# q8888620002/Group-Attribution-for-Diffusion-Models

Measured on AMD Instinct MI355X. Metric: shapley_coalitions_per_hour, higher is better.
Workload: dtype f32; 1 GPU; CIFAR-20 DDPM sFT coalition (BASELINE configs[1]): gd_steps=1000 @B=128 + 10240 samples x 100 DDIM steps @B=32 (32 batches fused/launch), UNet2DModel widths [128, 256, 256, 256] 35.75M params fp32; step = 1/1000 coalition = 1 train step + 1 sampler step @B=1024, enqueued on 3 HIP streams (the train step belongs to a later coalition: independent work); coalitions_in_flight=3

## Files before the change

### group-attribution-for-diffusion-models_amd/csrc/gemm_f32.hip

```cpp
#include "gad_common.h"
#include "gemm_dev.h"

using namespace gadk;

namespace gadk {
void launch_wino4_fused(const DevArgs& w, int bm, hipStream_t st);
}

namespace {

template <int ROWS, int VEC>
struct LoadKCDense : KCSlots<ROWS> {
  using S = KCSlots<ROWS>;
  const float* base;
  long roff[S::NS];
  unsigned rowmask;
  int kend, k;
  bool kok;
  __device__ void init(const float* b, int ld, int row0, int nrows, int kend_) {
    base = b;
    kend = kend_;
    rowmask = 0;
#pragma unroll
    for (int i = 0; i < S::NS; ++i) {
// ... 2009 lines not shown
    amul(d, col);
#pragma unroll
    for (int i = 0; i < 6; ++i) t[i][dx] = col[i];
  }
  const long pos_stride = p.T * p.C;
  float* out = p.V + tile * p.C + c;
#pragma unroll
  for (int i = 0; i < 6; ++i) {
    f32x4 v[6];
    amul(t[i], v);
#pragma unroll
    for (int j = 0; j < 6; ++j) *reinterpret_cast<f32x4*>(out + (long)(6 * i + j) * pos_stride) = v[j];
  }
}

__global__ __launch_bounds__(256) void wino4_dw_kernel(const float* dU, float* dW, int Cout, int Cin, int ldc) {
  const int C4 = Cin >> 2;
  const long idx = (long)blockIdx.x * 256 + threadIdx.x;
  if (idx >= (long)Cout * C4) return;
  const int co = (int)(idx / C4), ci = (int)(idx - (long)co * C4) * 4;
  const long ps = (long)Cout * Cin;
  const float* src = dU + (long)co * Cin + ci;
  auto gt = [](const f32x4 (&m)[6], f32x4 (&o)[3]) {
    const f32x4 s12 = m[1] + m[2], d21 = m[2] - m[1], s34 = m[3] + m[4], d34 = m[3] - m[4];
    o[0] = 0.25f * m[0] - (1.f / 6.f) * s12 + (1.f / 24.f) * s34;
    o[1] = (1.f / 6.f) * d21 + (1.f / 12.f) * d34;
    o[2] = (1.f / 6.f) * (s34 - s12) + m[5];
  };
  f32x4 t[3][6];
#pragma unroll
  for (int nu = 0; nu < 6; ++nu) {
    f32x4 m[6], col[3];
#pragma unroll
    for (int xi = 0; xi < 6; ++xi) m[xi] = ldg4(src + (long)(6 * xi + nu) * ps);
    gt(m, col);
#pragma unroll
    for (int r = 0; r < 3; ++r) t[r][nu] = col[r];
  }
  float* dst = dW + (long)co * ldc + ci;
#pragma unroll
  for (int r = 0; r < 3; ++r) {
    f32x4 o[3];
    gt(t[r], o);
#pragma unroll
    for (int sx = 0; sx < 3; ++sx) *reinterpret_cast<f32x4*>(dst + (long)(r * 3 + sx) * Cin) = o[sx];
  }
}

static FastDiv make_fastdiv(unsigned d) {
// ... 314 lines not shown
  out->lda = g.ldx;
  if (a->A2) {
    out->A_k2 = a->A2; out->lda_k2 = a->ldx2;
    out->B_k2 = a->B + a->a_split; out->ldb_k2 = a->ldb;
    out->k_split = a->a_split;
    out->A2 = nullptr; out->a_split = 0;
  }
  return true;
}
static gad_gemm_args canonical(const gad_gemm_args* a) {
  gad_gemm_args c;
  return as_dense_1x1(a, &c) ? c : *a;
}

constexpr int GAD_GEMM_INTERNAL_WINO4 = 1 << 30;
struct WinoPlan {
  int f;
  int fused4;
  int bm, bn, tiles_m, tiles_n;
  long T;
  int64_t bytes;
};
static bool use_wino(const gad_gemm_args* a, WinoPlan* wp) {
  const gad_conv_geom& g = a->g;
  if ((!a->B_wino && !a->B_wino4) || a->operand_precision != 0 || a->a_mode != GAD_A_CONV || a->b_mode != GAD_B_KC || a->A2 || a->A_k2) return false;
  if (!same_3x3(g) || (g.Ho & 1) || (g.Wo & 1)) return false;
  if (g.C % BK != 0 || g.ldx % 4 != 0 || a->N % 4 != 0 || a->N < 64 || (a->tile_hint != 0 && (a->tile_hint < HINT_WINO2 || a->tile_hint > HINT_WINO4_FUSED64)) || a->splitk_hint > 0 || a->batch > 1) return false;
  if (a->flags & (GAD_GEMM_NO_WINO | GAD_GEMM_NO_PATCH | GAD_GEMM_SCALAR_EPILOGUE | GAD_GEMM_TAP_MAJOR_K)) return false;
  if (a->rowadd && a->rows_per_group != g.Ho * g.Wo) return false;
  if (a->M % (g.Ho * g.Wo) != 0) return false;
// ... 252 lines not shown
extern "C" int gad_wino_weights(const float* src, float* dst, const int64_t* table, int64_t n_tiles, void* stream) {
  GAD_CHECK(src && dst && table && n_tiles > 0 && n_tiles < (1L << 31), "gad_wino_weights: bad arguments");
  static_assert(sizeof(long) == sizeof(int64_t), "table rows are 64-bit");
  hipLaunchKernelGGL(wino_weights_kernel, dim3((unsigned)n_tiles), dim3(256), 0, (hipStream_t)stream, src, dst, (const long*)table);
  GAD_LAUNCH_CHECK("gad_wino_weights");
  return 0;
}

extern "C" int gad_wino4_weights(const float* src, float* dst, const int64_t* table, int64_t n_tiles, void* stream) {
  GAD_CHECK(src && dst && table && n_tiles > 0 && n_tiles < (1L << 31), "gad_wino4_weights: bad arguments");
  hipLaunchKernelGGL(wino4_weights_kernel, dim3((unsigned)n_tiles), dim3(256), 0, (hipStream_t)stream, src, dst, (const long*)table);
  GAD_LAUNCH_CHECK("gad_wino4_weights");
  return 0;
}


static int check_args(const gad_gemm_args* a) {
  GAD_CHECK(a->M > 0 && a->N > 0 && a->K > 0, "gad_gemm: bad shape M=%d N=%d K=%d", a->M, a->N, a->K);
  const int am = a->a_mode, bmode = a->b_mode;
  GAD_CHECK(gad_aligned16(a->A) && gad_aligned16(a->B), "gad_gemm: A/B must be 16-byte aligned");
  const int k_first = a->A_k2 ? a->k_split : a->K;
  if (am == GAD_A_KC) GAD_CHECK(a->lda >= k_first, "gad_gemm: A_KC needs lda >= K (K=%d lda=%d)", k_first, a->lda);
  if (am == GAD_A_MC) GAD_CHECK(a->lda >= a->M, "gad_gemm: A_MC needs lda >= M (M=%d lda=%d)", a->M, a->lda);
  if (bmode == GAD_B_KC) GAD_CHECK(a->ldb >= k_first, "gad_gemm: B_KC needs ldb >= K (K=%d ldb=%d)", k_first, a->ldb);
  if (bmode == GAD_B_MC) GAD_CHECK(a->ldb >= a->N, "gad_gemm: B_MC needs ldb >= N (N=%d ldb=%d)", a->N, a->ldb);
  const bool convA = am == GAD_A_CONV || am == GAD_A_CONVT;
  if (convA || bmode == GAD_B_CONV || bmode == GAD_B_WDGRAD) {
    const gad_conv_geom& g = a->g;
    GAD_CHECK(g.H > 0 && g.W > 0 && g.C > 0 && g.Ho > 0 && g.Wo > 0 && g.KH > 0 && g.KW > 0 && g.stride > 0 &&
              g.ldx >= (a->A2 ? a->a_split : g.C), "gad_gemm: bad conv geometry");
// ... 34 lines not shown
  }
  if (a->rowadd) GAD_CHECK(a->rows_per_group > 0 && a->ld_rowadd >= a->N, "gad_gemm: bad rowadd");
  if (a->residual) GAD_CHECK(a->ldr >= a->N, "gad_gemm: bad residual stride");
  GAD_CHECK(a->ldc >= a->N, "gad_gemm: ldc < N");
  GAD_CHECK(a->operand_precision == 0 || a->operand_precision == 1, "gad_gemm: operand_precision must be 0 (f32) or 1 (bf16 allowed)");
  return 0;
}

static int check_stage_flags(const Route& r) {
  const bool only_input = (r.a.flags & GAD_GEMM_WINO_ONLY_INPUT) != 0, skip_input = (r.a.flags & GAD_GEMM_WINO_SKIP_INPUT) != 0;
  GAD_CHECK(!(only_input && skip_input), "gad_gemm: GAD_GEMM_WINO_ONLY_INPUT and GAD_GEMM_WINO_SKIP_INPUT exclude each other");
  GAD_CHECK(!only_input || r.kind == RouteKind::WINO,
            "gad_gemm: GAD_GEMM_WINO_ONLY_INPUT on a launch that takes no Winograd forward route (kernel id %d)", report(r).kid);
  GAD_CHECK(!skip_input || r.kind == RouteKind::WINO || r.kind == RouteKind::WINO_WGRAD,
            "gad_gemm: GAD_GEMM_WINO_SKIP_INPUT on a launch that takes no Winograd route (kernel id %d)", report(r).kid);
  return 0;
}

static DevArgs dev_args(const gad_gemm_args* a) {
  DevArgs d;
  d.A = a->A; d.B = a->B; d.C = a->C;
  d.A2 = a->A2; d.a_split = a->a_split; d.ldx2 = a->ldx2;
  d.Ak2 = a->A_k2; d.Bk2 = a->B_k2; d.lda2 = a->lda_k2; d.ldb2 = a->ldb_k2; d.k_split = a->k_split;
  d.Bh = nullptr;
  d.M = a->M; d.N = a->N; d.K = a->K;
  d.lda = a->lda; d.ldb = a->ldb; d.ldc = a->ldc;
  d.batch_inner = a->batch_inner > 0 ? a->batch_inner : 1;
  d.sA0 = a->strideA0; d.sA1 = a->strideA1; d.sB0 = a->strideB0; d.sB1 = a->strideB1;
  d.sC0 = a->strideC0; d.sC1 = a->strideC1;
  d.g = a->g;
// ... 21 lines not shown
static int launch_wino_wgrad(const Route& r, void* stream) {
  const gad_gemm_args* a = &r.a;
  const WinoWgradPlan& wq = r.wq;
  const gad_conv_geom& g = a->g;
  hipStream_t st = (hipStream_t)stream;
  GAD_CHECK(a->wino_ws && a->wino_ws_bytes >= wq.bytes && gad_aligned16(a->wino_ws),
            "gad_gemm: Winograd weight-gradient workspace too small or misaligned (%lld < %lld)", (long long)a->wino_ws_bytes, (long long)wq.bytes);
  float* Wy = (float*)a->wino_ws;
  float* V = Wy + wq.wy_bytes / 4;
  float* dU = V + wq.v_bytes / 4;
  const bool have_v = (a->flags & GAD_GEMM_WINO_SKIP_INPUT) && a->B_wino4 != nullptr;
  if (have_v) {
    GAD_CHECK(gad_aligned16(a->B_wino4), "gad_gemm: the kept Winograd input image (B_wino4 of a weight-gradient launch) must be 16-byte aligned");
    V = const_cast<float*>(a->B_wino4);
  }
  WinoIn wy;
  wy.x = a->A; wy.V = Wy;
  wy.H = g.Ho; wy.W = g.Wo; wy.C = a->M; wy.ldx = a->lda; wy.up = 0;
  wy.TH = g.Ho / 4; wy.TW = g.Wo / 4; wy.T = wq.T;
  WinoIn wi;
  wi.x = a->B; wi.V = V;
  wi.H = g.H; wi.W = g.W; wi.C = g.C; wi.ldx = g.ldx; wi.up = g.upsample ? 1 : 0;
  wi.TH = wy.TH; wi.TW = wy.TW; wi.T = wq.T;
  const long iy = wq.T * (a->M / 4), ix = wq.T * (g.C / 4);
  GAD_CHECK(gad_ceil_div(iy, 256) < (1L << 31) && gad_ceil_div(ix, 256) < (1L << 31), "gad_gemm: Winograd transform grid too large");
  hipLaunchKernelGGL(wino4_dy_kernel, dim3((unsigned)gad_ceil_div(iy, 256)), dim3(256), 0, st, wy);
  if (!have_v) hipLaunchKernelGGL(wino4_input_kernel, dim3((unsigned)gad_ceil_div(ix, 256)), dim3(256), 0, st, wi);
  GAD_LAUNCH_CHECK("gad_gemm(winograd wgrad transforms)");
  const gad_gemm_args sub = wino_wgrad_products_args(a, wq, Wy, V, dU);
  if (const int rc = gad_gemm(&sub, stream)) return rc;
  const long items = (long)a->M * (g.C / 4);
  hipLaunchKernelGGL(wino4_dw_kernel, dim3((unsigned)gad_ceil_div(items, 256)), dim3(256), 0, st, dU, a->C, a->M, g.C, a->ldc);
  GAD_LAUNCH_CHECK("gad_gemm(winograd wgrad output transform)");
  return 0;
}

static int launch_wino(const Route& r, const DevArgs& d, void* stream) {
  const gad_gemm_args* a = &r.a;
  const WinoPlan& wp = r.wp;
  const gad_conv_geom& g = a->g;
  hipStream_t st = (hipStream_t)stream;
  GAD_CHECK(a->wino_ws && a->wino_ws_bytes >= wp.bytes && gad_aligned16(a->wino_ws) && gad_aligned16(wp.f == 2 ? a->B_wino : a->B_wino4),
            "gad_gemm: Winograd workspace too small or misaligned (%lld < %lld)", (long long)a->wino_ws_bytes, (long long)wp.bytes);
  WinoIn wi;
  wi.x = a->A; wi.V = (float*)a->wino_ws;
  wi.H = g.H; wi.W = g.W; wi.C = g.C; wi.ldx = g.ldx; wi.up = g.upsample ? 1 : 0;
  wi.TH = g.Ho / wp.f; wi.TW = g.Wo / wp.f; wi.T = wp.T;
// ... 218 lines not shown
    else if (vec == 4) launch_mode<AMODE, BMODE_, 4>(d, pl, st);                       \
    else launch_mode<AMODE, BMODE_, 1>(d, pl, st);                                     \
  } else
  GAD_CASE(GAD_A_KC, GAD_B_KC)
  GAD_CASE(GAD_A_KC, GAD_B_MC)
  GAD_CASE(GAD_A_MC, GAD_B_MC)
  GAD_CASE(GAD_A_CONV, GAD_B_KC)
  GAD_CASE(GAD_A_CONVT, GAD_B_WDGRAD)
  GAD_CASE(GAD_A_MC, GAD_B_CONV)
  {
    gad_set_error("gad_gemm: unsupported mode pair a_mode=%d b_mode=%d", am, bmode);
    return 1;
  }
#undef GAD_CASE
  GAD_LAUNCH_CHECK("gad_gemm");
  if (pl.splitk > 1) {
    launch_splitk_reduce(d, (int)batch, st);
    GAD_LAUNCH_CHECK("gad_gemm(splitk reduce)");
  }
  return 0;
}

extern "C" int gad_gemm(const gad_gemm_args* args, void* stream) {
  GAD_CHECK(args && args->A && args->B && args->C, "gad_gemm: null pointer");
  const gad_gemm_args canon = canonical(args);
  if (const int rc = check_args(&canon)) return rc;
  const Route r = route_of(&canon);
  if (const int rc = check_stage_flags(r)) return rc;
  hipStream_t st = (hipStream_t)stream;
  DevArgs d = dev_args(&r.a);
  switch (r.kind) {
// ... 17 lines not shown
```

### group-attribution-for-diffusion-models_amd/gad/_capi.py

```python
import ctypes as C
import os

_HERE = os.path.dirname(os.path.abspath(__file__))
LIB_PATH = os.path.join(_HERE, "libgad_hip.so")


class GadError(RuntimeError):
    pass


class ConvGeom(C.Structure):
    _fields_ = [("H", C.c_int32), ("W", C.c_int32), ("C", C.c_int32), ("ldx", C.c_int32),
                ("Ho", C.c_int32), ("Wo", C.c_int32), ("KH", C.c_int32), ("KW", C.c_int32),
                ("stride", C.c_int32), ("pad_t", C.c_int32), ("pad_l", C.c_int32), ("upsample", C.c_int32)]


class GemmArgs(C.Structure):
    _fields_ = [("A", C.c_void_p), ("B", C.c_void_p), ("C", C.c_void_p),
                ("a_mode", C.c_int32), ("b_mode", C.c_int32),
                ("M", C.c_int32), ("N", C.c_int32), ("K", C.c_int32),
                ("lda", C.c_int32), ("ldb", C.c_int32), ("ldc", C.c_int32),
                ("batch", C.c_int32), ("batch_inner", C.c_int32),
                ("strideA0", C.c_int64), ("strideA1", C.c_int64), ("strideB0", C.c_int64),
                ("strideB1", C.c_int64), ("strideC0", C.c_int64), ("strideC1", C.c_int64),
                ("g", ConvGeom),
                ("alpha", C.c_float), ("bias", C.c_void_p), ("rowadd", C.c_void_p),
                ("rows_per_group", C.c_int32), ("ld_rowadd", C.c_int32),
                ("residual", C.c_void_p), ("ldr", C.c_int32),
                ("ws", C.c_void_p), ("ws_bytes", C.c_int64),
                ("tile_hint", C.c_int32), ("splitk_hint", C.c_int32), ("operand_precision", C.c_int32),
                ("A2", C.c_void_p), ("a_split", C.c_int32), ("ldx2", C.c_int32), ("B_bf16", C.c_void_p),
                ("A_k2", C.c_void_p), ("B_k2", C.c_void_p), ("lda_k2", C.c_int32), ("ldb_k2", C.c_int32),
                ("k_split", C.c_int32), ("flags", C.c_int32),
                ("B_wino", C.c_void_p), ("wino_ws", C.c_void_p), ("wino_ws_bytes", C.c_int64), ("B_wino4", C.c_void_p)]


class GroupNormArgs(C.Structure):
    _fields_ = [("x", C.c_void_p), ("y", C.c_void_p), ("gamma", C.c_void_p), ("beta", C.c_void_p),
                ("mean", C.c_void_p), ("rstd", C.c_void_p), ("dy", C.c_void_p),
                ("dgamma", C.c_void_p), ("dbeta", C.c_void_p),
                ("B", C.c_int32), ("HW", C.c_int32), ("C", C.c_int32), ("G", C.c_int32),
                ("eps", C.c_float), ("silu", C.c_int32), ("ws", C.c_void_p), ("ws_bytes", C.c_int64),
                ("x2", C.c_void_p), ("C1", C.c_int32), ("flags", C.c_int32), ("dx_add", C.c_void_p)]


class AttentionArgs(C.Structure):
    _fields_ = [("q", C.c_void_p), ("k", C.c_void_p), ("v", C.c_void_p), ("o", C.c_void_p), ("lse", C.c_void_p),
                ("d_o", C.c_void_p), ("delta", C.c_void_p), ("dq", C.c_void_p), ("dk", C.c_void_p), ("dv", C.c_void_p),
                ("B", C.c_int32), ("heads", C.c_int32), ("Tq", C.c_int32), ("Tk", C.c_int32), ("d", C.c_int32),
# ... 38 lines not shown


class HGemmSegArgs(C.Structure):
    _fields_ = [("A", C.c_void_p), ("B", C.c_void_p), ("C", C.c_void_p), ("ws", C.c_void_p), ("ws_bytes", C.c_int64),
                ("c_seg_stride", C.c_int64), ("M", C.c_int32), ("N", C.c_int32), ("L", C.c_int32), ("S", C.c_int32),
                ("lda", C.c_int32), ("ldb", C.c_int32), ("ldc", C.c_int32), ("alpha", C.c_float), ("accumulate", C.c_int32),
                ("splitk_hint", C.c_int32)]


JL_NORMAL, JL_RADEMACHER = 0, 1

GEMM_NO_PATCH, GEMM_TAP_MAJOR_K, GEMM_SCALAR_EPILOGUE, GEMM_GENERAL_LOADERS, GN_TWO_PASS = 1, 2, 4, 8, 1
GEMM_NO_WINO = 16
GEMM_WINO_WGRAD = 32
GEMM_WINO_ONLY_INPUT, GEMM_WINO_SKIP_INPUT = 64, 128
A_KC, A_MC, A_CONV, A_CONVT = 0, 1, 2, 3
B_KC, B_MC, B_WDGRAD, B_CONV = 0, 1, 2, 3

_vp, _i32, _i64, _f32, _f64 = C.c_void_p, C.c_int32, C.c_int64, C.c_float, C.c_double

SIGNATURES = {
    "gad_version": (C.c_int, []),
    "gad_last_error": (C.c_char_p, []),
    "gad_gemm_workspace_bytes": (_i64, [C.POINTER(GemmArgs)]),
    "gad_gemm": (C.c_int, [C.POINTER(GemmArgs), _vp]),
    "gad_gemm_uses_bf16": (C.c_int, [C.POINTER(GemmArgs)]),
    "gad_gemm_kernel_id": (C.c_int, [C.POINTER(GemmArgs)]),
    "gad_gemm_wino_bytes": (_i64, [C.POINTER(GemmArgs)]),
    "gad_wino_weights": (C.c_int, [_vp, _vp, _vp, _i64, _vp]),
    "gad_wino4_weights": (C.c_int, [_vp, _vp, _vp, _i64, _vp]),
    "gad_groupnorm_one_pass": (C.c_int, [C.POINTER(GroupNormArgs)]),
    "gad_gemm_plan": (C.c_int, [C.POINTER(GemmArgs), C.POINTER(_i32), C.POINTER(_i32), C.POINTER(_i32)]),
    "gad_groupnorm_workspace_bytes": (_i64, [C.POINTER(GroupNormArgs)]),
    "gad_groupnorm_silu_fwd": (C.c_int, [C.POINTER(GroupNormArgs), _vp]),
    "gad_groupnorm_silu_bwd": (C.c_int, [C.POINTER(GroupNormArgs), _vp]),
    "gad_groupnorm_wino4_ok": (C.c_int, [C.POINTER(GroupNormArgs), C.c_int32]),
    "gad_groupnorm_silu_wino4": (C.c_int, [C.POINTER(GroupNormArgs), _vp, C.c_int32, _vp]),
    "gad_attention_supported": (C.c_int, [_i32]),
    "gad_attention_uses_bf16": (C.c_int, [C.POINTER(AttentionArgs), _i32]),
    "gad_attention_bwd_workspace_bytes": (_i64, [C.POINTER(AttentionArgs)]),
    "gad_attention_fwd": (C.c_int, [C.POINTER(AttentionArgs), _vp]),
    "gad_attention_bwd": (C.c_int, [C.POINTER(AttentionArgs), _vp]),
    "gad_softmax_fwd": (C.c_int, [_vp, _vp, _i64, _i32, _f32, _vp]),
    "gad_softmax_bwd": (C.c_int, [_vp, _vp, _vp, _i64, _i32, _f32, _vp]),
    "gad_layernorm_workspace_bytes": (_i64, [_i64, _i32]),
# ... 73 lines not shown
```

### group-attribution-for-diffusion-models_amd/gad/ops.py

```python
from __future__ import annotations

import ctypes as C
import math
from typing import Optional

import torch

from . import _capi
from ._capi import (A_CONV, A_CONVT, A_KC, A_MC, B_CONV, B_KC, B_MC, B_WDGRAD, AdamArgs, ConvGeom, GemmArgs,
                    GroupNormArgs, check)

_WS = {}
WS_BYTES = 1 << 30


def _stream():
    return C.c_void_p(torch.cuda.current_stream().cuda_stream)


_raw_stream = getattr(torch._C, "_cuda_getCurrentRawStream", None)


WS_OVERRIDE = [None]

# ... 85 lines not shown

    def __exit__(self, *exc):
        OPERAND_PRECISION[0] = self.prev
        return False


def set_operand_precision(name):
    OPERAND_PRECISION[0] = 0 if name in (None, "no", "f32", "fp32") else operand_precision("bf16" if name in ("fp16", "bf16") else name).value


def half_activations() -> bool:
    return OPERAND_PRECISION[0] == 2


KERNEL_FLAGS = {"gemm": 0, "gn": 0, "native_dgrad": False, "two_kernel_attn_bwd": False, "narrow_attn_fwd": False, "no_wino4": False,
                "no_gn_wino": False}


class kernel_flags:

    def __init__(self, no_patch=False, tap_major_k=False, gn_two_pass=False, scalar_epilogue=False, general_loaders=False,
                 native_dgrad=False, two_kernel_attn_bwd=False, narrow_attn_fwd=False, no_wino=False, no_wino4=False, no_gn_wino=False):
        self.native_dgrad, self.two_kernel_attn_bwd, self.narrow_attn_fwd, self.no_wino4 = native_dgrad, two_kernel_attn_bwd, narrow_attn_fwd, no_wino4
        self.no_gn_wino = no_gn_wino
        self.gemm = ((_capi.GEMM_NO_PATCH if no_patch else 0) | (_capi.GEMM_TAP_MAJOR_K if tap_major_k else 0)
                     | (_capi.GEMM_NO_WINO if no_wino else 0)
                     | (_capi.GEMM_SCALAR_EPILOGUE if scalar_epilogue else 0)
                     | (_capi.GEMM_GENERAL_LOADERS if general_loaders else 0))
        self.gn = _capi.GN_TWO_PASS if gn_two_pass else 0

    def __enter__(self):
        self.prev = dict(KERNEL_FLAGS)
        KERNEL_FLAGS["gemm"], KERNEL_FLAGS["gn"], KERNEL_FLAGS["native_dgrad"] = self.gemm, self.gn, self.native_dgrad
        KERNEL_FLAGS["two_kernel_attn_bwd"], KERNEL_FLAGS["narrow_attn_fwd"] = self.two_kernel_attn_bwd, self.narrow_attn_fwd
        KERNEL_FLAGS["no_wino4"] = self.no_wino4
        KERNEL_FLAGS["no_gn_wino"] = self.no_gn_wino
        return self

    def __exit__(self, *exc):
        KERNEL_FLAGS.update(self.prev)
        return False


SCRATCH_ALLOC = None
OUT_ALLOC = None
OUT_ALLOC_DT = None


ROUTE_STATS = None


# ... 1 lines not shown
    if SCRATCH_ALLOC is not None:
        return SCRATCH_ALLOC(kind, nbytes, device)
    return torch.empty(nbytes, dtype=torch.uint8, device=device)


def _out(shape, device):
    if OUT_ALLOC is not None:
        return OUT_ALLOC(tuple(shape), device)
    return torch.empty(tuple(shape), device=device, dtype=torch.float32)


def gemm_raw(A, B, Cout, a_mode, b_mode, M, N, K, lda, ldb, ldc, *, geom: Optional[ConvGeom] = None, alpha=1.0,
             bias=None, rowadd=None, rows_per_group=1, residual=None, ldr=0, batch=1, batch_inner=1,
             sA=(0, 0), sB=(0, 0), sC=(0, 0), tile_hint=0, splitk_hint=0, A2=None, a_split=0, B_bf16=None,
             A_k2=None, B_k2=None, k_split=0, B_wino=None, B_wino4=None, wino_wgrad=False, wino_input=None, force_f32=False,
             keep_v=None, wino_v=None):
    lib = _capi.load()
    ws = workspace(A.device)
    a = GemmArgs()
    a.A, a.B, a.C = A.data_ptr(), B.data_ptr(), Cout.data_ptr()
    a.a_mode, a.b_mode = a_mode, b_mode
    a.M, a.N, a.K = M, N, K
    a.lda, a.ldb, a.ldc = lda, ldb, ldc
    a.batch, a.batch_inner = batch, batch_inner
    a.strideA0, a.strideA1 = sA
    a.strideB0, a.strideB1 = sB
    a.strideC0, a.strideC1 = sC
    if geom is not None:
        a.g = geom
    a.alpha = alpha
    a.bias, a.rowadd, a.residual = _ptr(bias), _ptr(rowadd), _ptr(residual)
# ... 12 lines not shown
        a.A_k2, a.B_k2, a.k_split = A_k2.data_ptr(), B_k2.data_ptr(), k_split
        a.lda_k2, a.ldb_k2 = A_k2.shape[-1], B_k2.shape[-1]
    if B_wino is not None or B_wino4 is not None:
        a.B_wino, a.B_wino4 = _ptr(B_wino), _ptr(B_wino4)
        need = lib.gad_gemm_wino_bytes(C.byref(a))
        if need:
            V = _scratch("wino", need, A.device)
            a.wino_ws, a.wino_ws_bytes = V.data_ptr(), need
            if keep_v is not None and a.B_wino4 and lib.gad_gemm_kernel_id(C.byref(a)) == 6:
                keep_v.append(V)
        else:
            a.B_wino = a.B_wino4 = None
    if wino_wgrad:
        a.flags |= _capi.GEMM_WINO_WGRAD
        need = lib.gad_gemm_wino_bytes(C.byref(a))
        if need:
            V = _scratch("wino", need, A.device)
            a.wino_ws, a.wino_ws_bytes = V.data_ptr(), need
            if wino_v is not None and wino_v.numel() >= 36 * (K // 16) * geom.C * 4:
                a.B_wino4 = wino_v.data_ptr()
                a.flags |= _capi.GEMM_WINO_SKIP_INPUT
        else:
            a.flags &= ~_capi.GEMM_WINO_WGRAD
    if wino_input is not None:
        if lib.gad_gemm_kernel_id(C.byref(a)) != 6 or not a.wino_ws:
            return False
        wino_input(V)
        a.flags |= _capi.GEMM_WINO_SKIP_INPUT
    if ROUTE_STATS is not None and (a.B_wino4 or a.flags & _capi.GEMM_WINO_WGRAD):
        key = (lib.gad_gemm_kernel_id(C.byref(a)), M, N, K, bool(a.flags & _capi.GEMM_WINO_SKIP_INPUT), torch.is_grad_enabled())
        ROUTE_STATS[key] = ROUTE_STATS.get(key, 0) + 1
    if SCRATCH_ALLOC is not None:
        need = lib.gad_gemm_workspace_bytes(C.byref(a))
        ws = _scratch("ws", need, A.device) if need else None
        a.ws, a.ws_bytes = (ws.data_ptr() if need else None), need
    if PROFILER is not None:
        PROFILER.gemm(lib, a, batch)
        return True
# ... 354 lines not shown
        gemm_raw(dy, wk, dxe, A_KC, B_MC, Bn * H * W, Cin, Cout, Cout, Cin, Cin, tile_hint=tile_hint, splitk_hint=splitk_hint)
        return dxe
    g = ConvGeom(Ho, Wo, Cout, Cout, He, We, KH, KW, stride, pad[0], pad[2], 0)
    gemm_raw(dy, wk, dxe, A_CONVT, B_WDGRAD, Bn * He * We, Cin, KH * KW * Cout, 0, 0, Cin, geom=g,
             tile_hint=tile_hint, splitk_hint=splitk_hint)
    return _upsample2x_bwd(dxe, x_shape) if upsample else dxe


def _upsample2x_bwd(dxe, x_shape):
    Bn, H, W, Cin = x_shape
    dx = torch.empty((Bn, H, W, Cin), device=dxe.device, dtype=torch.float32)
    check(_capi.load().gad_upsample2x_bwd(dxe.data_ptr(), dx.data_ptr(), Bn, H, W, Cin, _stream()), "gad_upsample2x_bwd")
    return dx


def conv2d_wgrad_raw(dy, x, w_like, stride=1, pad=(1, 1, 1, 1), upsample=False, tile_hint=0, splitk_hint=0, out=None, wino_v=None):
    _req(dy, "conv dy")
    _req(x, "conv x")
    Bn, H, W, Cin = x.shape
    Cout, _, KH, KW = w_like.shape
    _, Ho, Wo, _ = dy.shape
    dwk = _out((Cout, KH, KW, Cin), dy.device) if out is None else weight_krsc(out)
    if (KH == 1 and KW == 1 and stride == 1 and tuple(pad) == (0, 0, 0, 0) and not upsample and Cin % 4 == 0 and Cout % 4 == 0
            and not KERNEL_FLAGS["gemm"] & _capi.GEMM_GENERAL_LOADERS):
        gemm_raw(dy, x, dwk, A_MC, B_MC, Cout, Cin, Bn * H * W, Cout, Cin, Cin, tile_hint=tile_hint, splitk_hint=splitk_hint)
        return dwk.permute(0, 3, 1, 2)
    g = ConvGeom(H, W, Cin, Cin, Ho, Wo, KH, KW, stride, pad[0], pad[2], int(upsample))
    wino = (KH == 3 and KW == 3 and stride == 1 and tuple(pad) == (1, 1, 1, 1) and tile_hint in (0, 8) and splitk_hint == 0
            and Ho % 4 == 0 and Wo % 4 == 0 and OPERAND_PRECISION[0] == 0 and not KERNEL_FLAGS.get("no_wino4")
            and not KERNEL_FLAGS["gemm"] & (_capi.GEMM_NO_WINO | _capi.GEMM_NO_PATCH | _capi.GEMM_SCALAR_EPILOGUE | _capi.GEMM_TAP_MAJOR_K
                                            | _capi.GEMM_GENERAL_LOADERS))
    gemm_raw(dy, x, dwk, A_MC, B_CONV, Cout, KH * KW * Cin, Bn * Ho * Wo, Cout, 0, KH * KW * Cin, geom=g,
             tile_hint=tile_hint, splitk_hint=splitk_hint, wino_wgrad=wino, wino_v=wino_v)
    return dwk.permute(0, 3, 1, 2)


def colsum_raw(dy2d: torch.Tensor, segments=1, out=None):
    lib = _capi.load()
    ws = workspace(dy2d.device)
    rows, N = dy2d.shape
    if out is None:
        out = torch.empty((segments, N), device=dy2d.device, dtype=torch.float32)
    check(lib.gad_colsum(dy2d.data_ptr(), out.data_ptr(), segments, rows // segments, N, ws.data_ptr(), ws.numel(),
                         _stream()), "gad_colsum")
    return out


def linear_fwd_raw(x2d, w, bias=None, residual=None, alpha=1.0):
    M, K = x2d.shape
# ... 20 lines not shown


def _param_grad(param, compute):
    v, first = _sink(param)
    if v is None:
        return compute(None)
    if first:
        compute(v)
    else:
        v.add_(compute(None))
    return None


def _conv_backward(ctx, dy, x, x_shape, w, stride, pad, upsample, has, need):
    dy = dy.contiguous()
    dx = None
    if need[0]:
        if dgrad_as_forward(w, stride, pad):
            dx = conv2d_fwd_raw(dy, rotated_weight(w), None)
            if upsample:
                dx = _upsample2x_bwd(dx, x_shape)
        else:
            dx = conv2d_dgrad_raw(dy, w, x_shape, stride, pad, upsample)
    V, ctx.wino_v = ctx.wino_v, None
    dw = _param_grad(w, lambda o: conv2d_wgrad_raw(dy, x, w, stride, pad, upsample, out=o, wino_v=V)) if need[1] else None
    db, dr = _conv_epilogue_grads(dy, ctx.bias_ref, has[0] and need[2], has[1] and need[3])
    dres = dy if (has[2] and need[4]) else None
    return dx, dw, db, dr, dres


class Conv2dFn(torch.autograd.Function):

    @staticmethod
    def forward(ctx, x, w, bias, rowadd, residual, stride, pad, upsample):
        ctx.save_for_backward(x, w)
        ctx.bias_ref = bias
        ctx.cfg = (stride, pad, upsample, (bias is not None, rowadd is not None, residual is not None))
        keep = [] if ctx.needs_input_grad[1] else None
        y = conv2d_fwd_raw(x, w, bias, stride, pad, upsample, rowadd, residual, keep_v=keep)
        ctx.wino_v = keep[0] if keep else None
        return y

    @staticmethod
    def backward(ctx, dy):
        x, w = ctx.saved_tensors
        stride, pad, upsample, has = ctx.cfg
        return (*_conv_backward(ctx, dy, x, x.shape, w, stride, pad, upsample, has, ctx.needs_input_grad[:5]), None, None, None)


def _conv_epilogue_grads(dy, bias, need_bias, need_rowadd):
    Bn, Ho, Wo, Cout = dy.shape
    db = dr = None
    if need_rowadd:
        dr = colsum_raw(dy.view(Bn * Ho * Wo, Cout), segments=Bn)
        if need_bias:
            db = _param_grad(bias, lambda o: colsum_raw(dr, 1, out=o).view(Cout))
    elif need_bias:
        db = _param_grad(bias, lambda o: colsum_raw(dy.view(Bn * Ho * Wo, Cout), 1, out=o).view(Cout))
    return db, dr


class GnSiluConv3x3Fn(torch.autograd.Function):

    @staticmethod
    def forward(ctx, x, gamma, beta, w, bias, rowadd, residual, G, eps, bypass):
        _req(x, "groupnorm x")
        Bn = x.shape[0]
        mean = torch.empty((Bn, G), device=x.device, dtype=torch.float32)
# ... 752 lines not shown
```

### include/gad.h

```cpp
#ifndef GAD_H
#define GAD_H
#include <stdint.h>
#ifdef __cplusplus
extern "C" {
#endif

int gad_version(void);
const char* gad_last_error(void);

enum gad_a_mode {
  GAD_A_KC = 0,
  GAD_A_MC = 1,
  GAD_A_CONV = 2,
  GAD_A_CONVT = 3
};
enum gad_b_mode {
  GAD_B_KC = 0,
  GAD_B_MC = 1,
  GAD_B_WDGRAD = 2,
  GAD_B_CONV = 3
};

typedef struct gad_conv_geom {
  int32_t H, W, C;
// ... 25 lines not shown
  int64_t ws_bytes;
  int32_t tile_hint;
  int32_t splitk_hint;
  int32_t operand_precision;
  const float* A2;
  int32_t a_split, ldx2;
  const void* B_bf16;
  const float* A_k2;
  const float* B_k2;
  int32_t lda_k2, ldb_k2, k_split;
  int32_t flags;
  const float* B_wino;
  void* wino_ws;
  int64_t wino_ws_bytes;
  const float* B_wino4;
} gad_gemm_args;
enum gad_gemm_flags {
  GAD_GEMM_NO_WINO = 16,
  GAD_GEMM_WINO_WGRAD = 32,
  GAD_GEMM_NO_PATCH = 1,
  GAD_GEMM_TAP_MAJOR_K = 2,
  GAD_GEMM_SCALAR_EPILOGUE = 4,
  GAD_GEMM_GENERAL_LOADERS = 8,
  GAD_GEMM_WINO_ONLY_INPUT = 64,
  GAD_GEMM_WINO_SKIP_INPUT = 128
};

int64_t gad_gemm_workspace_bytes(const gad_gemm_args* a);
int gad_gemm_plan(const gad_gemm_args* a, int32_t* tile, int32_t* splitk, int32_t* vec);
int gad_gemm(const gad_gemm_args* a, void* stream);
int gad_gemm_uses_bf16(const gad_gemm_args* a);
int gad_gemm_kernel_id(const gad_gemm_args* a);
int64_t gad_gemm_wino_bytes(const gad_gemm_args* a);
int gad_wino_weights(const float* src, float* dst, const int64_t* table, int64_t n_tiles, void* stream);
int gad_wino4_weights(const float* src, float* dst, const int64_t* table, int64_t n_tiles, void* stream);

typedef struct gad_groupnorm_args {
  const float* x;
  float* y;
  const float* gamma;
  const float* beta;
  float* mean;
  float* rstd;
  const float* dy;
  float* dgamma;
  float* dbeta;
  int32_t B, HW, C, G;
  float eps;
  int32_t silu;
  void* ws;
// ... 187 lines not shown
```

Baseline: 44.90 coalitions/hour.

## Fuse dy Winograd transforms and bias sums into one pass; fold split-K into wgrad output

Adds a single kernel that reads dy once and produces three things: the Winograd input transform used by the dgrad-as-forward conv, the Winograd dy transform used by the weight-gradient route, and per-chunk channel partial sums that replace the bias and rowadd column sums. The weight-gradient launch can then skip its own dy transform. When the wgrad products GEMM uses split-K, the separate split-K reduce kernel is skipped and the slabs are summed inside the Winograd output-transform kernel. This removes several full passes over dy and one reduction launch. In exchange it needs an extra scratch buffer and more registers per thread in the fused kernel, and it adds a more complex control path in the Python backward.

Measured after the change: 45.26 coalitions/hour (median of 6 runs). Within noise of the previous version (+0.8%).

```diff
diff --git a/group-attribution-for-diffusion-models_amd/csrc/gemm_f32.hip b/group-attribution-for-diffusion-models_amd/csrc/gemm_f32.hip
--- a/group-attribution-for-diffusion-models_amd/csrc/gemm_f32.hip
+++ b/group-attribution-for-diffusion-models_amd/csrc/gemm_f32.hip
@@ -2047,12 +2047,107 @@
   }
 }
 
-__global__ __launch_bounds__(256) void wino4_dw_kernel(const float* dU, float* dW, int Cout, int Cin, int ldc) {
+constexpr int DYP_TL = 8, DYP_CQ = 32;
+struct WinoDyPass {
+  const float* dy;
+  float* Vd;
+  float* Wy;
+  float* part;
+  int H, W, C, ldx, TH, TW, P, cblocks;
+  long T;
+};
+
+__device__ __forceinline__ void wino4_a(const f32x4 (&d)[4], f32x4 (&t)[6]) {
+  const f32x4 s02 = d[0] + d[2], s13 = d[1] + d[3], a = d[0] + 4.f * d[2], b = 2.f * d[1] + 8.f * d[3];
+  t[0] = d[0];
+  t[1] = s02 + s13;
+  t[2] = s02 - s13;
+  t[3] = a + b;
+  t[4] = a - b;
+  t[5] = d[3];
+}
+
+__global__ __launch_bounds__(256) void wino4_dy_pass_kernel(const WinoDyPass p) {
+  __shared__ f32x4 red[DYP_TL][DYP_CQ];
+  const int tid = threadIdx.x, lane = tid / DYP_CQ, ql = tid - lane * DYP_CQ;
+  const int chunk = blockIdx.x / p.cblocks, cb = blockIdx.x - chunk * p.cblocks;
+  const int n = blockIdx.y, per = p.TH * p.TW;
+  const int r = chunk * DYP_TL + lane, cq = cb * DYP_CQ + ql, c = cq * 4;
+  const bool valid = r < per && c < p.C;
+  f32x4 s = zero4();
+  if (valid) {
+    const long tile = (long)n * per + r;
+    const int ty = r / p.TW, tx = r - ty * p.TW;
+    const float* img = p.dy + (long)n * p.H * p.W * p.ldx + c;
+    f32x4 t[6][6];
+    f32x4 in[4][4];
+#pragma unroll
+    for (int dx = 0; dx < 6; ++dx) {
+      const int xx = 4 * tx - 1 + dx;
+      const bool xok = xx >= 0 && xx < p.W;
+      f32x4 d[6], col[6];
+#pragma unroll
+      for (int dy = 0; dy < 6; ++dy) {
+        const int yy = 4 * ty - 1 + dy;
+        const bool ok = xok && yy >= 0 && yy < p.H;
+        d[dy] = ok ? ldg4(img + ((long)yy * p.W + xx) * p.ldx) : zero4();
+      }
+      wino4_bt(d, col);
+#pragma unroll
+      for (int i = 0; i < 6; ++i) t[i][dx] = col[i];
+      if (dx >= 1 && dx <= 4) {
+#pragma unroll
+        for (int dy = 0; dy < 4; ++dy) in[dy][dx - 1] = d[dy + 1];
+      }
+    }
+    const long pos_stride = p.T * p.C;
+    float* out = p.Vd + tile * p.C + c;
+#pragma unroll
+    for (int i = 0; i < 6; ++i) {
+      f32x4 v[6];
+      wino4_bt(t[i], v);
+#pragma unroll
+      for (int j = 0; j < 6; ++j) *reinterpret_cast<f32x4*>(out + (long)(6 * i + j) * pos_stride) = v[j];
+    }
+    f32x4 ta[6][4];
+#pragma unroll
+    for (int dx = 0; dx < 4; ++dx) {
+      f32x4 d[4], col[6];
+#pragma unroll
+      for (int dy = 0; dy < 4; ++dy) {
+        d[dy] = in[dy][dx];
+        s += d[dy];
+      }
+      wino4_a(d, col);
+#pragma unroll
+      for (int i = 0; i < 6; ++i) ta[i][dx] = col[i];
+    }
+    out = p.Wy + tile * p.C + c;
+#pragma unroll
+    for (int i = 0; i < 6; ++i) {
+      f32x4 v[6];
+      wino4_a(ta[i], v);
+#pragma unroll
+      for (int j = 0; j < 6; ++j) *reinterpret_cast<f32x4*>(out + (long)(6 * i + j) * pos_stride) = v[j];
+    }
+  }
+  red[lane][ql] = s;
+  __syncthreads();
+  if (lane == 0 && c < p.C) {
+    f32x4 v = red[0][ql];
+#pragma unroll
+    for (int l = 1; l < DYP_TL; ++l) v += red[l][ql];
+    *reinterpret_cast<f32x4*>(p.part + ((long)n * p.P + chunk) * p.C + c) = v;
+  }
+}
+
+template <bool SLABS>
+__global__ __launch_bounds__(256) void wino4_dw_kernel(const float* dU, float* dW, int Cout, int Cin, int ldc, int splitk) {
   const int C4 = Cin >> 2;
   const long idx = (long)blockIdx.x * 256 + threadIdx.x;
   if (idx >= (long)Cout * C4) return;
   const int co = (int)(idx / C4), ci = (int)(idx - (long)co * C4) * 4;
-  const long ps = (long)Cout * Cin;
+  const long mn = (long)Cout * Cin, ps = SLABS ? mn * splitk : mn;
   const float* src = dU + (long)co * Cin + ci;
   auto gt = [](const f32x4 (&m)[6], f32x4 (&o)[3]) {
     const f32x4 s12 = m[1] + m[2], d21 = m[2] - m[1], s34 = m[3] + m[4], d34 = m[3] - m[4];
@@ -2065,7 +2160,16 @@
   for (int nu = 0; nu < 6; ++nu) {
     f32x4 m[6], col[3];
 #pragma unroll
-    for (int xi = 0; xi < 6; ++xi) m[xi] = ldg4(src + (long)(6 * xi + nu) * ps);
+    for (int xi = 0; xi < 6; ++xi) {
+      const float* w = src + (long)(6 * xi + nu) * ps;
+      if constexpr (SLABS) {
+        f32x4 v = zero4();
+        for (int sl = 0; sl < splitk; ++sl) v += ldg4(w + (long)sl * mn);
+        m[xi] = v;
+      } else {
+        m[xi] = ldg4(w);
+      }
+    }
     gt(m, col);
 #pragma unroll
     for (int r = 0; r < 3; ++r) t[r][nu] = col[r];
@@ -2410,6 +2514,7 @@
 }
 
 constexpr int GAD_GEMM_INTERNAL_WINO4 = 1 << 30;
+constexpr int GAD_GEMM_INTERNAL_KEEP_SLABS = 1 << 29;
 struct WinoPlan {
   int f;
   int fused4;
@@ -2692,6 +2797,30 @@
   return 0;
 }
 
+extern "C" int32_t gad_wino4_dy_pass_parts(int32_t H, int32_t W) {
+  if (H <= 0 || W <= 0 || (H & 3) || (W & 3)) return 0;
+  return (int32_t)gad_ceil_div((long)(H / 4) * (W / 4), DYP_TL);
+}
+
+extern "C" int gad_wino4_dy_pass(const float* dy, float* Vd, float* Wy, float* part, int32_t B, int32_t H, int32_t W, int32_t C,
+                                 int32_t ldx, void* stream) {
+  GAD_CHECK(dy && Vd && Wy && part, "gad_wino4_dy_pass: null pointer");
+  GAD_CHECK(gad_aligned16(dy) && gad_aligned16(Vd) && gad_aligned16(Wy) && gad_aligned16(part), "gad_wino4_dy_pass: pointers must be 16-byte aligned");
+  GAD_CHECK(B > 0 && B < 65536 && H > 0 && W > 0 && !(H & 3) && !(W & 3) && C > 0 && C % 4 == 0 && ldx >= C && ldx % 4 == 0,
+            "gad_wino4_dy_pass: bad shape B=%d H=%d W=%d C=%d ldx=%d (maps multiples of 4, C %% 4 == 0)", B, H, W, C, ldx);
+  GAD_CHECK((long)H * W * ldx < (1L << 31), "gad_wino4_dy_pass: image too large for 32-bit pixel offsets");
+  WinoDyPass p;
+  p.dy = dy; p.Vd = Vd; p.Wy = Wy; p.part = part;
+  p.H = H; p.W = W; p.C = C; p.ldx = ldx;
+  p.TH = H / 4; p.TW = W / 4; p.T = (long)B * p.TH * p.TW;
+  p.P = gad_wino4_dy_pass_parts(H, W);
+  p.cblocks = (int)gad_ceil_div(C / 4, DYP_CQ);
+  GAD_CHECK((long)p.P * p.cblocks < (1L << 31), "gad_wino4_dy_pass: grid too large");
+  hipLaunchKernelGGL(wino4_dy_pass_kernel, dim3((unsigned)(p.P * p.cblocks), (unsigned)B), dim3(256), 0, (hipStream_t)stream, p);
+  GAD_LAUNCH_CHECK("gad_wino4_dy_pass");
+  return 0;
+}
+
 
 static int check_args(const gad_gemm_args* a) {
   GAD_CHECK(a->M > 0 && a->N > 0 && a->K > 0, "gad_gemm: bad shape M=%d N=%d K=%d", a->M, a->N, a->K);
@@ -2756,6 +2885,8 @@
             "gad_gemm: GAD_GEMM_WINO_ONLY_INPUT on a launch that takes no Winograd forward route (kernel id %d)", report(r).kid);
   GAD_CHECK(!skip_input || r.kind == RouteKind::WINO || r.kind == RouteKind::WINO_WGRAD,
             "gad_gemm: GAD_GEMM_WINO_SKIP_INPUT on a launch that takes no Winograd route (kernel id %d)", report(r).kid);
+  GAD_CHECK(!(r.a.flags & GAD_GEMM_WINO_SKIP_DY) || r.kind == RouteKind::WINO_WGRAD,
+            "gad_gemm: GAD_GEMM_WINO_SKIP_DY on a launch that does not take the Winograd weight-gradient route (kernel id %d)", report(r).kid);
   return 0;
 }
 
@@ -2807,6 +2938,13 @@
     GAD_CHECK(gad_aligned16(a->B_wino4), "gad_gemm: the kept Winograd input image (B_wino4 of a weight-gradient launch) must be 16-byte aligned");
     V = const_cast<float*>(a->B_wino4);
   }
+  const bool have_wy = (a->flags & GAD_GEMM_WINO_SKIP_DY) != 0;
+  if (have_wy) {
+    GAD_CHECK(a->dy_wino4 && gad_aligned16(a->dy_wino4) && a->dy_wino4_bytes >= wq.wy_bytes,
+              "gad_gemm: the supplied Winograd dy image (GAD_GEMM_WINO_SKIP_DY) is null, misaligned or too small (%lld < %lld bytes)",
+              (long long)a->dy_wino4_bytes, (long long)wq.wy_bytes);
+    Wy = const_cast<float*>(a->dy_wino4);
+  }
   WinoIn wy;
   wy.x = a->A; wy.V = Wy;
   wy.H = g.Ho; wy.W = g.Wo; wy.C = a->M; wy.ldx = a->lda; wy.up = 0;
@@ -2817,13 +2955,18 @@
   wi.TH = wy.TH; wi.TW = wy.TW; wi.T = wq.T;
   const long iy = wq.T * (a->M / 4), ix = wq.T * (g.C / 4);
   GAD_CHECK(gad_ceil_div(iy, 256) < (1L << 31) && gad_ceil_div(ix, 256) < (1L << 31), "gad_gemm: Winograd transform grid too large");
-  hipLaunchKernelGGL(wino4_dy_kernel, dim3((unsigned)gad_ceil_div(iy, 256)), dim3(256), 0, st, wy);
+  if (!have_wy) hipLaunchKernelGGL(wino4_dy_kernel, dim3((unsigned)gad_ceil_div(iy, 256)), dim3(256), 0, st, wy);
   if (!have_v) hipLaunchKernelGGL(wino4_input_kernel, dim3((unsigned)gad_ceil_div(ix, 256)), dim3(256), 0, st, wi);
   GAD_LAUNCH_CHECK("gad_gemm(winograd wgrad transforms)");
-  const gad_gemm_args sub = wino_wgrad_products_args(a, wq, Wy, V, dU);
+  gad_gemm_args sub = wino_wgrad_products_args(a, wq, Wy, V, dU);
+  const Route rs = route_of(&sub);
+  const int slabs = rs.kind == RouteKind::ENGINE && rs.plan.splitk > 1 && gad_aligned16(a->ws) && !(a->flags & GAD_GEMM_WINO_WGRAD_REDUCE) ? rs.plan.splitk : 1;
+  if (slabs > 1) sub.flags |= GAD_GEMM_INTERNAL_KEEP_SLABS;
   if (const int rc = gad_gemm(&sub, stream)) return rc;
   const long items = (long)a->M * (g.C / 4);
-  hipLaunchKernelGGL(wino4_dw_kernel, dim3((unsigned)gad_ceil_div(items, 256)), dim3(256), 0, st, dU, a->C, a->M, g.C, a->ldc);
+  const dim3 dgrid((unsigned)gad_ceil_div(items, 256));
+  if (slabs > 1) hipLaunchKernelGGL(wino4_dw_kernel<true>, dgrid, dim3(256), 0, st, (const float*)a->ws, a->C, a->M, g.C, a->ldc, slabs);
+  else hipLaunchKernelGGL(wino4_dw_kernel<false>, dgrid, dim3(256), 0, st, (const float*)dU, a->C, a->M, g.C, a->ldc, 1);
   GAD_LAUNCH_CHECK("gad_gemm(winograd wgrad output transform)");
   return 0;
 }
@@ -3072,7 +3215,7 @@
   }
 #undef GAD_CASE
   GAD_LAUNCH_CHECK("gad_gemm");
-  if (pl.splitk > 1) {
+  if (pl.splitk > 1 && !(a->flags & GAD_GEMM_INTERNAL_KEEP_SLABS)) {
     launch_splitk_reduce(d, (int)batch, st);
     GAD_LAUNCH_CHECK("gad_gemm(splitk reduce)");
   }
diff --git a/group-attribution-for-diffusion-models_amd/gad/_capi.py b/group-attribution-for-diffusion-models_amd/gad/_capi.py
--- a/group-attribution-for-diffusion-models_amd/gad/_capi.py
+++ b/group-attribution-for-diffusion-models_amd/gad/_capi.py
@@ -32,7 +32,8 @@
                 ("A2", C.c_void_p), ("a_split", C.c_int32), ("ldx2", C.c_int32), ("B_bf16", C.c_void_p),
                 ("A_k2", C.c_void_p), ("B_k2", C.c_void_p), ("lda_k2", C.c_int32), ("ldb_k2", C.c_int32),
                 ("k_split", C.c_int32), ("flags", C.c_int32),
-                ("B_wino", C.c_void_p), ("wino_ws", C.c_void_p), ("wino_ws_bytes", C.c_int64), ("B_wino4", C.c_void_p)]
+                ("B_wino", C.c_void_p), ("wino_ws", C.c_void_p), ("wino_ws_bytes", C.c_int64), ("B_wino4", C.c_void_p),
+                ("dy_wino4", C.c_void_p), ("dy_wino4_bytes", C.c_int64)]
 
 
 class GroupNormArgs(C.Structure):
@@ -101,6 +102,8 @@
 GEMM_NO_WINO = 16
 GEMM_WINO_WGRAD = 32
 GEMM_WINO_ONLY_INPUT, GEMM_WINO_SKIP_INPUT = 64, 128
+GEMM_WINO_SKIP_DY = 256
+GEMM_WINO_WGRAD_REDUCE = 512
 A_KC, A_MC, A_CONV, A_CONVT = 0, 1, 2, 3
 B_KC, B_MC, B_WDGRAD, B_CONV = 0, 1, 2, 3
 
@@ -116,6 +119,8 @@
     "gad_gemm_wino_bytes": (_i64, [C.POINTER(GemmArgs)]),
     "gad_wino_weights": (C.c_int, [_vp, _vp, _vp, _i64, _vp]),
     "gad_wino4_weights": (C.c_int, [_vp, _vp, _vp, _i64, _vp]),
+    "gad_wino4_dy_pass_parts": (_i32, [_i32, _i32]),
+    "gad_wino4_dy_pass": (C.c_int, [_vp, _vp, _vp, _vp, _i32, _i32, _i32, _i32, _i32, _vp]),
     "gad_groupnorm_one_pass": (C.c_int, [C.POINTER(GroupNormArgs)]),
     "gad_gemm_plan": (C.c_int, [C.POINTER(GemmArgs), C.POINTER(_i32), C.POINTER(_i32), C.POINTER(_i32)]),
     "gad_groupnorm_workspace_bytes": (_i64, [C.POINTER(GroupNormArgs)]),
diff --git a/group-attribution-for-diffusion-models_amd/gad/ops.py b/group-attribution-for-diffusion-models_amd/gad/ops.py
--- a/group-attribution-for-diffusion-models_amd/gad/ops.py
+++ b/group-attribution-for-diffusion-models_amd/gad/ops.py
@@ -123,19 +123,22 @@
 
 
 KERNEL_FLAGS = {"gemm": 0, "gn": 0, "native_dgrad": False, "two_kernel_attn_bwd": False, "narrow_attn_fwd": False, "no_wino4": False,
-                "no_gn_wino": False}
+                "no_gn_wino": False, "no_dy_pass": False}
 
 
 class kernel_flags:
 
     def __init__(self, no_patch=False, tap_major_k=False, gn_two_pass=False, scalar_epilogue=False, general_loaders=False,
-                 native_dgrad=False, two_kernel_attn_bwd=False, narrow_attn_fwd=False, no_wino=False, no_wino4=False, no_gn_wino=False):
+                 native_dgrad=False, two_kernel_attn_bwd=False, narrow_attn_fwd=False, no_wino=False, no_wino4=False, no_gn_wino=False,
+                 no_dy_pass=False):
+        self.no_dy_pass = no_dy_pass
         self.native_dgrad, self.two_kernel_attn_bwd, self.narrow_attn_fwd, self.no_wino4 = native_dgrad, two_kernel_attn_bwd, narrow_attn_fwd, no_wino4
         self.no_gn_wino = no_gn_wino
         self.gemm = ((_capi.GEMM_NO_PATCH if no_patch else 0) | (_capi.GEMM_TAP_MAJOR_K if tap_major_k else 0)
                      | (_capi.GEMM_NO_WINO if no_wino else 0)
                      | (_capi.GEMM_SCALAR_EPILOGUE if scalar_epilogue else 0)
-                     | (_capi.GEMM_GENERAL_LOADERS if general_loaders else 0))
+                     | (_capi.GEMM_GENERAL_LOADERS if general_loaders else 0)
+                     | (_capi.GEMM_WINO_WGRAD_REDUCE if no_dy_pass else 0))
         self.gn = _capi.GN_TWO_PASS if gn_two_pass else 0
 
     def __enter__(self):
@@ -144,6 +147,7 @@
         KERNEL_FLAGS["two_kernel_attn_bwd"], KERNEL_FLAGS["narrow_attn_fwd"] = self.two_kernel_attn_bwd, self.narrow_attn_fwd
         KERNEL_FLAGS["no_wino4"] = self.no_wino4
         KERNEL_FLAGS["no_gn_wino"] = self.no_gn_wino
+        KERNEL_FLAGS["no_dy_pass"] = self.no_dy_pass
         return self
 
     def __exit__(self, *exc):
@@ -175,7 +179,7 @@
              bias=None, rowadd=None, rows_per_group=1, residual=None, ldr=0, batch=1, batch_inner=1,
              sA=(0, 0), sB=(0, 0), sC=(0, 0), tile_hint=0, splitk_hint=0, A2=None, a_split=0, B_bf16=None,
              A_k2=None, B_k2=None, k_split=0, B_wino=None, B_wino4=None, wino_wgrad=False, wino_input=None, force_f32=False,
-             keep_v=None, wino_v=None):
+             keep_v=None, wino_v=None, wino_dy=None, wino_query=False):
     lib = _capi.load()
     ws = workspace(A.device)
     a = GemmArgs()
@@ -218,14 +222,24 @@
     if wino_wgrad:
         a.flags |= _capi.GEMM_WINO_WGRAD
         need = lib.gad_gemm_wino_bytes(C.byref(a))
+        if wino_query:
+            return need
         if need:
-            V = _scratch("wino", need, A.device)
+            wy_bytes = 36 * (K // 16) * M * 4
+            if wino_dy is not None and wino_dy.numel() >= need:
+                V = wino_dy
+                a.dy_wino4, a.dy_wino4_bytes = V.data_ptr(), wy_bytes
+                a.flags |= _capi.GEMM_WINO_SKIP_DY
+            else:
+                V = _scratch("wino", need, A.device)
             a.wino_ws, a.wino_ws_bytes = V.data_ptr(), need
             if wino_v is not None and wino_v.numel() >= 36 * (K // 16) * geom.C * 4:
                 a.B_wino4 = wino_v.data_ptr()
                 a.flags |= _capi.GEMM_WINO_SKIP_INPUT
         else:
             a.flags &= ~_capi.GEMM_WINO_WGRAD
+    if wino_query:
+        return 0
     if wino_input is not None:
         if lib.gad_gemm_kernel_id(C.byref(a)) != 6 or not a.wino_ws:
             return False
@@ -610,15 +624,21 @@
     return dx
 
 
-def conv2d_wgrad_raw(dy, x, w_like, stride=1, pad=(1, 1, 1, 1), upsample=False, tile_hint=0, splitk_hint=0, out=None, wino_v=None):
+def conv2d_wgrad_raw(dy, x, w_like, stride=1, pad=(1, 1, 1, 1), upsample=False, tile_hint=0, splitk_hint=0, out=None, wino_v=None,
+                     wino_dy=None, wino_query=False):
     _req(dy, "conv dy")
     _req(x, "conv x")
     Bn, H, W, Cin = x.shape
     Cout, _, KH, KW = w_like.shape
     _, Ho, Wo, _ = dy.shape
-    dwk = _out((Cout, KH, KW, Cin), dy.device) if out is None else weight_krsc(out)
+    if wino_query:
+        dwk = dy if out is None else weight_krsc(out)
+    else:
+        dwk = _out((Cout, KH, KW, Cin), dy.device) if out is None else weight_krsc(out)
     if (KH == 1 and KW == 1 and stride == 1 and tuple(pad) == (0, 0, 0, 0) and not upsample and Cin % 4 == 0 and Cout % 4 == 0
             and not KERNEL_FLAGS["gemm"] & _capi.GEMM_GENERAL_LOADERS):
+        if wino_query:
+            return 0
         gemm_raw(dy, x, dwk, A_MC, B_MC, Cout, Cin, Bn * H * W, Cout, Cin, Cin, tile_hint=tile_hint, splitk_hint=splitk_hint)
         return dwk.permute(0, 3, 1, 2)
     g = ConvGeom(H, W, Cin, Cin, Ho, Wo, KH, KW, stride, pad[0], pad[2], int(upsample))
@@ -626,9 +646,22 @@
             and Ho % 4 == 0 and Wo % 4 == 0 and OPERAND_PRECISION[0] == 0 and not KERNEL_FLAGS.get("no_wino4")
             and not KERNEL_FLAGS["gemm"] & (_capi.GEMM_NO_WINO | _capi.GEMM_NO_PATCH | _capi.GEMM_SCALAR_EPILOGUE | _capi.GEMM_TAP_MAJOR_K
                                             | _capi.GEMM_GENERAL_LOADERS))
-    gemm_raw(dy, x, dwk, A_MC, B_CONV, Cout, KH * KW * Cin, Bn * Ho * Wo, Cout, 0, KH * KW * Cin, geom=g,
-             tile_hint=tile_hint, splitk_hint=splitk_hint, wino_wgrad=wino, wino_v=wino_v)
-    return dwk.permute(0, 3, 1, 2)
+    res = gemm_raw(dy, x, dwk, A_MC, B_CONV, Cout, KH * KW * Cin, Bn * Ho * Wo, Cout, 0, KH * KW * Cin, geom=g,
+                   tile_hint=tile_hint, splitk_hint=splitk_hint, wino_wgrad=wino, wino_v=wino_v, wino_dy=wino_dy, wino_query=wino_query)
+    return res if wino_query else dwk.permute(0, 3, 1, 2)
+
+
+def wino4_dy_pass_raw(dy, Vd, Wy):
+    lib = _capi.load()
+    Bn, Ho, Wo, Cout = dy.shape
+    P = lib.gad_wino4_dy_pass_parts(Ho, Wo)
+    img = 36 * (Bn * Ho * Wo // 16) * Cout * 4
+    if not P or Vd.numel() < img or Wy.numel() < img:
+        raise _capi.GadError(f"wino4_dy_pass: dy {tuple(dy.shape)} needs maps that are multiples of 4 and {img} bytes per image")
+    part = _out((Bn, P, Cout), dy.device)
+    check(lib.gad_wino4_dy_pass(dy.data_ptr(), Vd.data_ptr(), Wy.data_ptr(), part.data_ptr(), Bn, Ho, Wo, Cout, Cout, _stream()),
+          "gad_wino4_dy_pass")
+    return part
 
 
 def colsum_raw(dy2d: torch.Tensor, segments=1, out=None):
@@ -679,17 +712,27 @@
 
 def _conv_backward(ctx, dy, x, x_shape, w, stride, pad, upsample, has, need):
     dy = dy.contiguous()
-    dx = None
+    dx = part = Wy = None
     if need[0]:
         if dgrad_as_forward(w, stride, pad):
-            dx = conv2d_fwd_raw(dy, rotated_weight(w), None)
+            if need[1] and not upsample and not KERNEL_FLAGS.get("no_dy_pass"):
+                sink = getattr(w, "_gad_sink", None) if _SINK_ACTIVE[0] else None
+                wy_need = conv2d_wgrad_raw(dy, x, w, stride, pad, upsample, out=sink, wino_query=True)
+                if wy_need:
+                    def fill(Vd):
+                        nonlocal part, Wy
+                        Wy = _scratch("wino", wy_need, dy.device)
+                        part = wino4_dy_pass_raw(dy, Vd, Wy)
+                    dx = conv2d_fwd_raw(_ShapeOnly(dy, dy.shape), rotated_weight(w), None, wino_input=fill)
+            if dx is None:
+                dx = conv2d_fwd_raw(dy, rotated_weight(w), None)
             if upsample:
                 dx = _upsample2x_bwd(dx, x_shape)
         else:
             dx = conv2d_dgrad_raw(dy, w, x_shape, stride, pad, upsample)
     V, ctx.wino_v = ctx.wino_v, None
-    dw = _param_grad(w, lambda o: conv2d_wgrad_raw(dy, x, w, stride, pad, upsample, out=o, wino_v=V)) if need[1] else None
-    db, dr = _conv_epilogue_grads(dy, ctx.bias_ref, has[0] and need[2], has[1] and need[3])
+    dw = _param_grad(w, lambda o: conv2d_wgrad_raw(dy, x, w, stride, pad, upsample, out=o, wino_v=V, wino_dy=Wy)) if need[1] else None
+    db, dr = _conv_epilogue_grads(dy, ctx.bias_ref, has[0] and need[2], has[1] and need[3], part)
     dres = dy if (has[2] and need[4]) else None
     return dx, dw, db, dr, dres
 
@@ -713,10 +756,17 @@
         return (*_conv_backward(ctx, dy, x, x.shape, w, stride, pad, upsample, has, ctx.needs_input_grad[:5]), None, None, None)
 
 
-def _conv_epilogue_grads(dy, bias, need_bias, need_rowadd):
+def _conv_epilogue_grads(dy, bias, need_bias, need_rowadd, part=None):
     Bn, Ho, Wo, Cout = dy.shape
     db = dr = None
-    if need_rowadd:
+    if part is not None and (need_bias or need_rowadd):
+        P = part.shape[1]
+        dr = part.view(Bn, Cout) if P == 1 else colsum_raw(part.view(Bn * P, Cout), segments=Bn)
+        if need_bias:
+            db = _param_grad(bias, lambda o: colsum_raw(dr, 1, out=o).view(Cout))
+        if not need_rowadd:
+            dr = None
+    elif need_rowadd:
         dr = colsum_raw(dy.view(Bn * Ho * Wo, Cout), segments=Bn)
         if need_bias:
             db = _param_grad(bias, lambda o: colsum_raw(dr, 1, out=o).view(Cout))
diff --git a/include/gad.h b/include/gad.h
--- a/include/gad.h
+++ b/include/gad.h
@@ -63,6 +63,8 @@
   void* wino_ws;
   int64_t wino_ws_bytes;
   const float* B_wino4;
+  const float* dy_wino4;
+  int64_t dy_wino4_bytes;
 } gad_gemm_args;
 enum gad_gemm_flags {
   GAD_GEMM_NO_WINO = 16,
@@ -72,7 +74,9 @@
   GAD_GEMM_SCALAR_EPILOGUE = 4,
   GAD_GEMM_GENERAL_LOADERS = 8,
   GAD_GEMM_WINO_ONLY_INPUT = 64,
-  GAD_GEMM_WINO_SKIP_INPUT = 128
+  GAD_GEMM_WINO_SKIP_INPUT = 128,
+  GAD_GEMM_WINO_SKIP_DY = 256,
+  GAD_GEMM_WINO_WGRAD_REDUCE = 512
 };
 
 int64_t gad_gemm_workspace_bytes(const gad_gemm_args* a);
@@ -83,6 +87,9 @@
 int64_t gad_gemm_wino_bytes(const gad_gemm_args* a);
 int gad_wino_weights(const float* src, float* dst, const int64_t* table, int64_t n_tiles, void* stream);
 int gad_wino4_weights(const float* src, float* dst, const int64_t* table, int64_t n_tiles, void* stream);
+int32_t gad_wino4_dy_pass_parts(int32_t H, int32_t W);
+int gad_wino4_dy_pass(const float* dy, float* Vd, float* Wy, float* part, int32_t B, int32_t H, int32_t W, int32_t C, int32_t ldx,
+                      void* stream);
 
 typedef struct gad_groupnorm_args {
   const float* x;
```
